# BreakTheBeta/Zonos_Vibes

Measured on AMD Instinct MI355X. Metric: real-time factor (44kHz audio s/compute s) + DAC tokens/s/GPU, Zonos-transformer, higher is better.
Workload: dtype bf16; 1 GPU; C2: batch=1 per GPU, Lc=160, 861 frames (10.00 s audio), greedy + rep. penalty, EOS suppressed, + DAC decode; global_batch=1, seq_len=1030, parallelism=dp1 (utterance-sharded), decode_steps=869

## Files before the change

### zonos_vibes_amd/csrc/zmi_gemv_impl.h

```cpp
#pragma once
#include <algorithm>
#include "zmi_common.h"
#include "zmi_kernels.h"
#include "zmi_gemv_row.h"
#include "zmi_rownorm.h"

namespace zmi_gemv {

constexpr int PRO_PLAIN = 0, PRO_LN = 1, PRO_ADDLN = 2, PRO_GRMS = 3;
constexpr int PRO_GRMSG = 4;
constexpr size_t LDS_MAX = 160 * 1024;

__device__ __forceinline__ void dma_piece(const bf16_t* gsrc, bf16_t* ldp) {
  const unsigned ldst =
      __builtin_amdgcn_readfirstlane((unsigned)(size_t)(__attribute__((address_space(3))) void*)ldp);
  unsigned keep;
  asm volatile("s_mov_b32 %0, m0\n\ts_mov_b32 m0, %2\n\ts_nop 0\n\tglobal_load_lds_dwordx4 %1, off\n\t"
               "s_mov_b32 m0, %0"
               : "=&s"(keep)
               : "v"(gsrc), "s"(ldst)
               : "memory");
}

template <int K>
struct Img {
  static constexpr int XROW = K + 8, GROW = K + 8;
  __host__ __device__ static constexpr bool grms(int pro) { return pro == PRO_GRMS || pro == PRO_GRMSG; }
  __host__ __device__ static constexpr size_t aux_off(int rows) { return (size_t)rows * XROW * 2; }
  __host__ __device__ static constexpr size_t gamma_off(int rows, int pro) {
    return aux_off(rows) + (size_t)rows * (pro == PRO_ADDLN ? XROW * 2 : (grms(pro) ? GROW * 4 : 0));
  }
  __host__ __device__ static constexpr size_t red_off(int rows, int pro) {
    return gamma_off(rows, pro) + (size_t)K * ((pro == PRO_LN || pro == PRO_ADDLN) ? 4 : (grms(pro) ? 2 : 0));
  }
  __host__ __device__ static constexpr size_t bytes(int rows, int nwv, int rt, int pro) {
    return red_off(rows, pro) + (size_t)nwv * 8 * rt * 4;
  }
  struct View {
    bf16_t *xs, *xa, *gam, *bet;
    float *xg, *red;
  };
  __device__ static View carve(char* smem, int rows, int pro) {
    char *aux = smem + aux_off(rows), *gamma = smem + gamma_off(rows, pro);
    return {reinterpret_cast<bf16_t*>(smem), reinterpret_cast<bf16_t*>(aux), reinterpret_cast<bf16_t*>(gamma),
            reinterpret_cast<bf16_t*>(gamma) + K, reinterpret_cast<float*>(aux),
            reinterpret_cast<float*>(smem + red_off(rows, pro))};
  }
};
template <int K>
using View = typename Img<K>::View;

#ifdef ZMI_GEMV_STAMPS
#define ZMI_GSTAMP(i)                                                                              \
  do {                                                                                             \
    __builtin_amdgcn_sched_barrier(0);                                                             \
    if (threadIdx.x == 0 && a.diag)                                                                \
      reinterpret_cast<unsigned long long*>(a.diag)[((size_t)a.reserved * 4096 + blockIdx.x) * 8 + (i)] = \
          __builtin_amdgcn_s_memrealtime();                                                        \
    __builtin_amdgcn_sched_barrier(0);                                                             \
  } while (0)
#else
#define ZMI_GSTAMP(i) \
  do {                \
  } while (0)
#endif

struct QkvFuse {
  uint64_t* gran;
  int gran_stride;
  int og_off = 0, of_off = 0, hkv = 0;
  const int* pos = nullptr;
  unsigned* err = nullptr;
  int l2_cols = 0;
};

__device__ __forceinline__ const float2* rope_pair(const ZmiGemvArgs& a, int q_pos, int n) {
  const int qcols = a.hq * a.hd, d = (n < qcols ? n : n - qcols) % a.hd;
  return reinterpret_cast<const float2*>(a.rope + ((size_t)q_pos * (a.hd >> 1) + (d >> 1)) * 2);
}

template <int EPI, int RT, int FUSE, class Sum>
__device__ __forceinline__ void epilogue(const ZmiGemvArgs& a, const Sum& colsum, int lane, int rows, int row0,
                                         int g, const uint32_t (&res_pre)[(8 * RT + 63) / 64], int q_pos, int q_kvr,
                                         const QkvFuse& fz, unsigned act_rows = ~0u, const float2* rope_pre = nullptr) {
  constexpr int NE = (8 * RT + 63) / 64;
  const int col0 = g * 8;
  if (EPI == ZMI_EPI_STORE && FUSE == 2) {
#pragma unroll
    for (int i = 0; i < NE; ++i) {
      const int e = lane + 64 * i, r = e >> 3, c = e & 7, n = col0 + c;
      const bool ok = r < rows && n < a.n_valid;
      const uint32_t hv = ok ? f2bf(colsum(c, r)) : 0u;
      const uint32_t nb = (uint32_t)__shfl_down((int)hv, 1);
      if (ok) {
        const size_t m = (size_t)(row0 + r);
        reinterpret_cast<bf16_t*>(a.out)[m * a.ldo + n] = (bf16_t)hv;
        const int pos = a.row_pos[m];
        if ((c & 1) == 0 && pos >= 0)
          st_xc64(fz.gran + m * fz.gran_stride + (n >> 1), (uint64_t)(hv | (nb << 16)) | ((uint64_t)(unsigned)(pos + 1) << 32),
                  n < fz.l2_cols);
      }
    }
  } else if (EPI == ZMI_EPI_STORE || EPI == ZMI_EPI_RESIDUAL || EPI == ZMI_EPI_F32 || EPI == ZMI_EPI_LOGITS) {
#pragma unroll
    for (int i = 0; i < NE; ++i) {
      const int e = lane + 64 * i, r = e >> 3, c = e & 7, n = col0 + c;
      if (r >= rows || n >= a.n_valid || !((act_rows >> r) & 1u)) continue;
      const float v = colsum(c, r);
      const size_t m = (size_t)(row0 + r);
      if (EPI == ZMI_EPI_F32) {
        reinterpret_cast<float*>(a.out)[m * a.ldo + n] = v;
      } else if (EPI == ZMI_EPI_STORE) {
        reinterpret_cast<bf16_t*>(a.out)[m * a.ldo + n] = (bf16_t)f2bf(v);
      } else if (EPI == ZMI_EPI_RESIDUAL) {
        reinterpret_cast<bf16_t*>(a.out)[m * a.ldo + n] = (bf16_t)f2bf(bf2f(res_pre[i]) + bfround(v));
      } else {
        const int cbk = n / 1026, vv = n - cbk * 1026;
        reinterpret_cast<float*>(a.out)[(m * 9 + cbk) * 1026 + vv] = bfround(v);
      }
    }
  } else if (EPI == ZMI_EPI_SWIGLU) {
    const int r = lane >> 2, c = lane & 3;
    if (r < rows) {
      const float y = bfround(colsum(c, r));
      const float gt = bfround(colsum(c + 4, r));
      const float sg = bfround(gt / (1.0f + expf(-gt)));
      reinterpret_cast<bf16_t*>(a.out)[(size_t)(row0 + r) * a.ldo + g * 4 + c] = (bf16_t)f2bf(y * sg);
    }
  } else if (EPI == ZMI_EPI_QKV) {
    const int r = lane >> 2, c = (lane & 3) * 2;
    if (r < rows && q_pos >= 0 && q_pos < a.smax) {
      const int n = col0 + c;
      const int qcols = a.hq * a.hd, kcols = a.hkv * a.hd;
      float x0 = bfround(colsum(c, r)), x1 = bfround(colsum(c + 1, r));
      if (n < qcols + kcols) {
        const float2 cs = rope_pre ? *rope_pre : *rope_pair(a, q_pos, n);
        const float co = cs.x, si = cs.y;
        const float r0 = x0 * co - x1 * si;
        const float r1 = x1 * co + x0 * si;
        x0 = r0;
        x1 = r1;
      }
      const uint32_t packed = f2bf(x0) | (f2bf(x1) << 16);
      int gkh = 0, gslot = 0;
      if (n < qcols) {
        *reinterpret_cast<uint32_t*>(reinterpret_cast<bf16_t*>(a.out) + (size_t)(row0 + r) * a.ldo + n) = packed;
        const int gq = a.hq / a.hkv;
        gkh = n / (gq * a.hd);
        gslot = (n - gkh * gq * a.hd) >> 1;
      } else if (n < qcols + kcols) {
        const int nn = n - qcols, kh = nn / a.hd, d = nn - kh * a.hd;
        const size_t o = (((size_t)q_kvr * a.hkv + kh) * a.smax + q_pos) * a.hd + d;
        *reinterpret_cast<uint32_t*>(reinterpret_cast<bf16_t*>(a.k_cache) + o) = packed;
        gkh = kh;
        gslot = (a.hq / a.hkv) * (a.hd >> 1) + (d >> 1);
      } else {
        const int nn = n - qcols - kcols, kh = nn / a.hd, d = nn - kh * a.hd;
        bf16_t* vt = reinterpret_cast<bf16_t*>(a.v_cache) + (((size_t)q_kvr * a.hkv + kh) * a.hd + d) * a.smax + q_pos;
        vt[0] = (bf16_t)(packed & 0xffffu);
        vt[a.smax] = (bf16_t)(packed >> 16);
        gkh = kh;
        gslot = (a.hq / a.hkv + 1) * (a.hd >> 1) + (d >> 1);
      }
      if (FUSE)
        st_wt64(fz.gran + ((size_t)(row0 + r) * a.hkv + gkh) * fz.gran_stride + gslot,
                (uint64_t)packed | ((uint64_t)(unsigned)(q_pos + 1) << 32));
    }
  }
}

template <int K, int PRO, int NWV>
__device__ __forceinline__ void stage_rows(const ZmiGemvArgs& a, const View<K>& L, int wave, int lane,
                                           bool first, int s_row0, int s_rows) {
  constexpr int XROW = Img<K>::XROW, GROW = Img<K>::GROW;
  constexpr bool GRMS = Img<K>::grms(PRO), AUX = PRO == PRO_ADDLN || GRMS;
  constexpr int GB = (PRO == PRO_LN || PRO == PRO_ADDLN) ? 2 : (GRMS ? 1 : 0);
  constexpr int PPR = K / 512;
  const int n_x = PRO == PRO_GRMSG ? 0 : s_rows * PPR;
  constexpr int APR = GRMS ? 2 * PPR : PPR;
  const int n_a = AUX ? s_rows * APR : 0;
  const int n_pc = n_x + n_a + (first ? GB * PPR : 0);
  const bf16_t* s_X = reinterpret_cast<const bf16_t*>(a.X) + (size_t)s_row0 * a.ldx;
  const bf16_t* XA = AUX ? reinterpret_cast<const bf16_t*>(a.aux) + (size_t)s_row0 * a.ld_aux * (GRMS ? 2 : 1)
                         : nullptr;
  for (int pc = wave; pc < n_pc; pc += NWV) {
    if (pc < n_x) {
      const int r = pc / PPR, p = pc - r * PPR;
      dma_piece(s_X + (size_t)r * a.ldx + p * 512 + lane * 8, L.xs + r * XROW + p * 512);
    } else if (pc < n_x + n_a) {
      const int r = (pc - n_x) / APR, p = (pc - n_x) - r * APR;
      if (GRMS)
        dma_piece(XA + ((size_t)r * a.ld_aux + p * 256) * 2 + lane * 8,
                  reinterpret_cast<bf16_t*>(L.xg + r * GROW + p * 256));
      else
        dma_piece(XA + (size_t)r * a.ld_aux + p * 512 + lane * 8, L.xa + r * XROW + p * 512);
    } else {
      const int q = pc - n_x - n_a, which = q / PPR, p = q - which * PPR;
      const bf16_t* src = reinterpret_cast<const bf16_t*>(which ? a.ln_b : a.ln_w);
      dma_piece(src + p * 512 + lane * 8, (which ? L.bet : L.gam) + p * 512);
    }
  }
}

template <int EPI, int RT>
__device__ __forceinline__ void stage_epilogue_operands(const ZmiGemvArgs& a, bool ew, int lane, int rows, int row0,
                                                        int col0, uint32_t (&res_pre)[(8 * RT + 63) / 64], int& q_pos,
                                                        int& q_kvr) {
  constexpr int NE = (8 * RT + 63) / 64;
#pragma unroll
  for (int i = 0; i < NE; ++i) res_pre[i] = 0;
  q_pos = -1, q_kvr = 0;
  if (EPI == ZMI_EPI_RESIDUAL && ew) {
#pragma unroll
    for (int i = 0; i < NE; ++i) {
      const int e = lane + 64 * i, r = e >> 3, n = col0 + (e & 7);
      if (r < rows && n < a.n_valid)
        res_pre[i] = reinterpret_cast<const bf16_t*>(a.out)[(size_t)(row0 + r) * a.ldo + n];
    }
  }
  if (EPI == ZMI_EPI_QKV && ew && (lane >> 2) < rows) {
    q_pos = a.row_pos[row0 + (lane >> 2)];
    q_kvr = a.row_kv[row0 + (lane >> 2)];
  }
}

template <int K, int NWV>
__device__ __forceinline__ unsigned gather_attention_rows(const ZmiGemvArgs& a, const QkvFuse& fz, bf16_t* xs, int* qpos,
                                                          int rows, int row0, int tid) {
  constexpr int XROW = Img<K>::XROW;
  const int lane = tid & 63, wave = __builtin_amdgcn_readfirstlane(tid >> 6);
  if (tid < rows) qpos[tid] = fz.pos[row0 + tid];
  __syncthreads();
  unsigned act_rows = 0u;
  for (int r = 0; r < rows; ++r) act_rows |= (qpos[r] >= 0 ? 1u : 0u) << r;
  const int n_units = rows * fz.hkv;
  if (wave == 0) {
    for (unsigned spins = 0;; ++spins) {
      bool ok = false;
      for (int u0 = 0; u0 < n_units; u0 += 8) {
        const int u = u0 + (lane >> 3), qp = u < n_units ? qpos[u / fz.hkv] : -1;
        const bool up = qp < 0 || (uint32_t)(ld_wt64(fz.gran + (size_t)(row0 * fz.hkv + u) * fz.gran_stride + fz.of_off +
                                                        (lane & 7)) >> 32) == (uint32_t)qp + 1u;
        float f = up ? 1.f : 0.f;
        f = fmaxf(f, dpp_mov<DPP_XOR1>(f));
        f = fmaxf(f, dpp_mov<DPP_XOR2>(f));
        f = fmaxf(f, dpp_mov<DPP_HALF_MIRROR>(f));
        ok = ok || (u < n_units && f > 0.f);
      }
      if (__any(ok)) break;
      if (spins > (1u << 18)) {
        if (lane == 0) __hip_atomic_store(fz.err, 1u, __ATOMIC_RELAXED, __HIP_MEMORY_SCOPE_AGENT);
        break;
      }
      __builtin_amdgcn_s_sleep(2);
    }
  }
  ZMI_GSTAMP(7);
  __syncthreads();
  constexpr int GPT = 4;
  for (int e0 = tid; e0 < n_units * 256; e0 += GPT * NWV * 64) {
    uint64_t gv[GPT];
    int gq[GPT];
    unsigned need = 0;
#pragma unroll
    for (int i = 0; i < GPT; ++i) {
      const int e = e0 + NWV * 64 * i;
      gq[i] = e < n_units * 256 ? qpos[(e >> 8) / fz.hkv] : -1;
      gv[i] = 0ull;
      if (gq[i] >= 0) need |= 1u << i;
    }
    for (unsigned spins = 0; need; ++spins) {
#pragma unroll
      for (int i = 0; i < GPT; ++i)
        if ((need >> i) & 1)
          gv[i] = ld_wt64(fz.gran + (size_t)(row0 * fz.hkv + ((e0 + NWV * 64 * i) >> 8)) * fz.gran_stride + fz.og_off +
                          ((e0 + NWV * 64 * i) & 255));
#pragma unroll
      for (int i = 0; i < GPT; ++i)
        if (((need >> i) & 1) && (uint32_t)(gv[i] >> 32) == (uint32_t)gq[i] + 1u) need &= ~(1u << i);
      if (!need) break;
      if (spins > (1u << 18)) {
        __hip_atomic_store(fz.err, 1u, __ATOMIC_RELAXED, __HIP_MEMORY_SCOPE_AGENT);
        break;
      }
      __builtin_amdgcn_s_sleep(1);
    }
#pragma unroll
    for (int i = 0; i < GPT; ++i) {
      const int e = e0 + NWV * 64 * i;
      if (e < n_units * 256) {
        const int u = e >> 8, j = e & 255, r = u / fz.hkv, kh = u - r * fz.hkv;
        *reinterpret_cast<uint32_t*>(xs + r * XROW + kh * 512 + 2 * j) = gq[i] >= 0 ? (uint32_t)gv[i] : 0u;
      }
    }
  }
  return act_rows;
}

template <int K, int RT, int NWV, bool ADD>
__device__ __forceinline__ void ln_statistics(const ZmiGemvArgs& a, const View<K>& L, int rows, int wave, int lane) {
  constexpr int XROW = Img<K>::XROW, NQ = ln_parts(K), CPQ = ln_chunks(K);
  float* part = L.red;
  const int ntask = rows * NQ;
  auto pass = [&](int task, float mean, bool sq) {
    const int r = task / NQ, q = task - r * NQ;
    float t = 0.f;
#pragma unroll
    for (int i = 0; i < CPQ; ++i) {
      const int off = r * XROW + ln_chunk_off(K, q, lane, i);
      const uint4 xv = ld_chunk(L.xs + off);
      if constexpr (ADD)
        t += addln_chunk_sum(xv, ld_chunk(L.xa + off), mean, sq);
      else
        t += ln_chunk_sum(xv, mean, sq);
    }
    return wave_sum(t);
  };
  for (int task = wave; task < ntask; task += NWV) {
    const float v = pass(task, 0.f, false);
    if (lane == 0) part[task] = v;
  }
  __syncthreads();
#if defined(ZMI_LN_STAMP) && ZMI_LN_STAMP == 1
  ZMI_GSTAMP(7);
#endif
  for (int task = wave; task < ntask; task += NWV) {
    const float mean = ln_combine<NQ>(part + (task / NQ) * NQ) / (float)K;
    const float v = pass(task, mean, true);
    if (lane == 0) part[RT * NQ + task] = v;
  }
  __syncthreads();
#if defined(ZMI_LN_STAMP) && ZMI_LN_STAMP == 2
  ZMI_GSTAMP(7);
#endif
}

template <int K, int RT, int NWV>
__device__ __forceinline__ void prologue_layernorm(const ZmiGemvArgs& a, const View<K>& L, int rows, int wave, int lane) {
  constexpr int XROW = Img<K>::XROW, NQ = ln_parts(K), CPQ = ln_chunks(K);
  ln_statistics<K, RT, NWV, false>(a, L, rows, wave, lane);
  for (int task = wave; task < rows * NQ; task += NWV) {
    const int r = task / NQ, q = task - r * NQ;
    const float mean = ln_combine<NQ>(L.red + r * NQ) / (float)K;
    const float rstd = 1.0f / sqrtf(ln_combine<NQ>(L.red + RT * NQ + r * NQ) / (float)K + a.eps), nbias = -mean * rstd;
#pragma unroll
    for (int i = 0; i < CPQ; ++i) {
      const int off = ln_chunk_off(K, q, lane, i);
      bf16_t* xp = L.xs + r * XROW + off;
      st_chunk(xp, ln_apply(ld_chunk(xp), ld_chunk(L.gam + off), ld_chunk(L.bet + off), rstd, nbias));
    }
  }
  __syncthreads();
}

template <int K, int RT, int NWV>
__device__ __forceinline__ void prologue_add_layernorm(const ZmiGemvArgs& a, const View<K>& L, int rows,
                                                       int row0, bool wres, int wave, int lane) {
  constexpr int XROW = Img<K>::XROW, NQ = ln_parts(K), CPQ = ln_chunks(K);
  ln_statistics<K, RT, NWV, true>(a, L, rows, wave, lane);
  for (int task = wave; task < rows * NQ; task += NWV) {
    const int r = task / NQ, q = task - r * NQ;
    const float mean = ln_combine<NQ>(L.red + r * NQ) / (float)K;
    const float rstd = 1.0f / sqrtf(ln_combine<NQ>(L.red + RT * NQ + r * NQ) / (float)K + a.eps);
#pragma unroll
    for (int i = 0; i < CPQ; ++i) {
      const int off = ln_chunk_off(K, q, lane, i);
      bf16_t* hp = L.xs + r * XROW + off;
      const AddLnChunk o = addln_apply(ld_chunk(hp), ld_chunk(L.xa + r * XROW + off), ld_chunk(L.gam + off),
                                       ld_chunk(L.bet + off), mean, rstd);
      st_chunk(hp, o.y);
      if (wres) st_chunk(reinterpret_cast<bf16_t*>(a.res_out) + (size_t)(row0 + r) * a.ld_aux + off, o.s);
    }
  }
  __syncthreads();
}

template <int K, int RT, int NWV, int PRO>
__device__ __forceinline__ void prologue_gated_rmsnorm(const ZmiGemvArgs& a, const View<K>& L, int rows,
                                                       int wave, int lane) {
  constexpr int XROW = Img<K>::XROW, GROW = Img<K>::GROW, NQ = ln_parts(K), CPQ = ln_chunks(K);
  float* part = L.red;
  const int ntask = rows * NQ;
  auto load_g = [&](int r, int off, float (&g)[8]) {
    uint32_t y[4] = {0u, 0u, 0u, 0u};
    if constexpr (PRO == PRO_GRMS) {
      const uint4 yv = *reinterpret_cast<const uint4*>(L.xs + r * XROW + off);
      y[0] = yv.x; y[1] = yv.y; y[2] = yv.z; y[3] = yv.w;
    }
    float gz[8];
    load_gate(L.xg + r * GROW + off, gz);
#pragma unroll
    for (int e = 0; e < 8; ++e) g[e] = PRO == PRO_GRMSG ? gz[e] : gate_elem(y, gz, e);
  };
  for (int task0 = wave; task0 < ntask; task0 += 2 * NWV) {
    float t[2];
#pragma unroll
    for (int u = 0; u < 2; ++u) {
      const int task = min(task0 + u * NWV, ntask - 1);
      const int r = task / NQ, q = task - r * NQ;
      t[u] = 0.f;
#pragma unroll
      for (int i = 0; i < CPQ; ++i) {
        float g[8];
        load_g(r, ln_chunk_off(K, q, lane, i), g);
        t[u] = grms_chunk_sq(g, t[u]);
      }
    }
#pragma unroll
    for (int u = 0; u < 2; ++u) t[u] = wave_sum(t[u]);
    if (lane == 0) {
      part[task0] = t[0];
      if (task0 + NWV < ntask) part[task0 + NWV] = t[1];
    }
  }
  __syncthreads();
  for (int task0 = wave; task0 < ntask; task0 += 2 * NWV) {
    uint4 res[2][CPQ];
#pragma unroll
    for (int u = 0; u < 2; ++u) {
      const int task = min(task0 + u * NWV, ntask - 1);
      const int r = task / NQ, q = task - r * NQ;
      const float rstd = 1.0f / sqrtf(ln_combine<NQ>(part + r * NQ) / (float)K + a.eps);
#pragma unroll
      for (int i = 0; i < CPQ; ++i) {
        const int off = ln_chunk_off(K, q, lane, i);
        const uint4 gw = *reinterpret_cast<const uint4*>(L.gam + off);
        float g[8];
        load_g(r, off, g);
        res[u][i] = grms_apply(g, gw, rstd);
      }
    }
#pragma unroll
    for (int u = 0; u < 2; ++u) {
      const int task = task0 + u * NWV;
      if (task < ntask) {
        const int r = task / NQ, q = task - r * NQ;
        bf16_t* yr = L.xs + r * XROW;
#pragma unroll
        for (int i = 0; i < CPQ; ++i) *reinterpret_cast<uint4*>(yr + ln_chunk_off(K, q, lane, i)) = res[u][i];
      }
    }
  }
  __syncthreads();
}

template <int G, int W, int NL, int RT, int PRO, int EPI, int NTW, int FUSE = 0, int FMT = ZMI_WFMT_BF16>
__device__ __forceinline__ void gemv_body(const ZmiGemvArgs& a, int n_cb, int n_rt, int b, char* smem,
                                          const QkvFuse& fz, int rpw = 1) {
  constexpr int K = W * NL * 64;
  constexpr int KC = K / 64;
  constexpr int NWV = G * W;
  constexpr int XROW = Img<K>::XROW;
  constexpr bool F8 = FMT == ZMI_WFMT_FP8;
  constexpr int CHB = F8 ? 512 : 1024;
  constexpr int NWL = F8 ? NL / 2 : NL;
  static_assert(FMT == ZMI_WFMT_BF16 || F8, "weight format");
  static_assert(!F8 || (NL % 2 == 0 && FUSE == 0 && (PRO == PRO_PLAIN || PRO == PRO_LN)),
                "fp8 weights: the MLP projections' plain / LayerNorm launches");
  static_assert(RT == 8 || RT == 16, "row tile");
  static_assert(!FUSE || EPI == ZMI_EPI_QKV || EPI == ZMI_EPI_STORE || FUSE == 3, "in-launch hand-off: QKV or plain store");
  static_assert(FUSE != 2 || NTW, "the store hand-off runs on single-tile (decode) launches");
  static_assert(FUSE != 3 || (NTW && (EPI == ZMI_EPI_RESIDUAL || EPI == ZMI_EPI_STORE) && PRO == PRO_PLAIN && K == 2048 &&
                              RT == 16),
                "the gathered-input form is zmi_attn_block's out_proj role (one tile, plain, residual or store epilogue)");

  const auto [cb, rg] = block_pos(b, n_rt, rpw);
  if (cb >= n_cb) return;
  ZMI_GSTAMP(0);
  int rt = rg * rpw;
  const int rt_end = min(n_rt, rt + rpw);
  int row0 = rt * RT;
  int rows = min(RT, a.M - row0);
  const View<K> L = Img<K>::carve(smem, a.M < RT ? a.M : RT, PRO);

  const int tid = threadIdx.x, lane = tid & 63;
  const int wave = __builtin_amdgcn_readfirstlane(tid >> 6);
  const int gi = wave / W, wk = wave - gi * W;
  const int ngroups = a.N >> 3;
  const int g_raw = cb * G + gi;
  const bool g_ok = g_raw < ngroups;
  const int g = g_ok ? g_raw : ngroups - 1;
  const int col0 = g * 8;
  const bool ew = (wk == 0) && g_ok;
  constexpr int NE = (8 * RT + 63) / 64;
  uint32_t res_pre[NE];
  int q_pos = -1, q_kvr = 0;
  unsigned act_rows = ~0u;

  if (FUSE != 3) stage_rows<K, PRO, NWV>(a, L, wave, lane, true, row0, rows);
  stage_epilogue_operands<EPI, RT>(a, ew, lane, rows, row0, col0, res_pre, q_pos, q_kvr);
  uint2 wexp = {0u, 0u};
  if constexpr (F8) {
    if (ew) wexp = *reinterpret_cast<const uint2*>(reinterpret_cast<const char*>(a.w_exp) + col0);
  }
  __builtin_amdgcn_sched_barrier(0);
  u32x4_t wf[NWL];
  load_weights_m8<NWL, NTW ? 2 : 0>(reinterpret_cast<const char*>(a.W) + ((size_t)g * KC + wk * NL) * CHB, NL * CHB,
                                    lane, wf);
  __builtin_amdgcn_sched_barrier(0);
  ZMI_GSTAMP(1);
  asm volatile("s_waitcnt vmcnt(%0)" ::"n"(NWL) : "memory");
  if constexpr (F8) {
    wexp.x = __builtin_amdgcn_readfirstlane(wexp.x);
    wexp.y = __builtin_amdgcn_readfirstlane(wexp.y);
  }
  float2 rope_cs = {1.f, 0.f};
  if (EPI == ZMI_EPI_QKV && NTW && ew && (lane >> 2) < rows && q_pos >= 0 && q_pos < a.smax) {
    const int n = col0 + (lane & 3) * 2;
    if (n < a.hq * a.hd + a.hkv * a.hd) rope_cs = *rope_pair(a, q_pos, n);
  }
  __builtin_amdgcn_sched_barrier(0);
  if constexpr (FUSE == 3)
    act_rows = gather_attention_rows<K, NWV>(a, fz, L.xs, reinterpret_cast<int*>(L.red), rows, row0, tid);
  for (;;) {
    __builtin_amdgcn_s_barrier();
    __builtin_amdgcn_sched_barrier(0);
    ZMI_GSTAMP(2);
    if constexpr (PRO == PRO_LN) prologue_layernorm<K, RT, NWV>(a, L, rows, wave, lane);
    if constexpr (PRO == PRO_ADDLN)
      prologue_add_layernorm<K, RT, NWV>(a, L, rows, row0, a.res_out != nullptr && cb == 0, wave, lane);
    if constexpr (PRO == PRO_GRMS || PRO == PRO_GRMSG) prologue_gated_rmsnorm<K, RT, NWV, PRO>(a, L, rows, wave, lane);
    ZMI_GSTAMP(3);

    f32x4_t acc0 = {0.f, 0.f, 0.f, 0.f}, acc1 = {0.f, 0.f, 0.f, 0.f};
    chain_m8<NL, F8>(L.xs + min(lane & 15, rows - 1) * XROW + wk * NL * 64 + (lane >> 4) * 8, wf, acc0, acc1);
    ZMI_GSTAMP(4);
    const SegPos sp = segment_pos<false>(lane);
#pragma unroll
    for (int q = 0; q < 4; ++q) {
      const float v = segment_value<false>(acc0, acc1, q);
      if (sp.live && sp.rb + q < RT) L.red[(wave * 8 + sp.c) * RT + sp.rb + q] = v;
    }
    __syncthreads();
    ZMI_GSTAMP(5);
    if (!NTW && rt + 1 < rt_end) {
      const int n_row0 = (rt + 1) * RT;
      stage_rows<K, PRO, NWV>(a, L, wave, lane, false, n_row0, min(RT, a.M - n_row0));
    }
    if (ew)
      epilogue<EPI, RT, FUSE>(a, ColSum<W, RT, F8>{L.red + gi * W * 8 * RT, wexp}, lane, rows, row0, g, res_pre, q_pos,
                              q_kvr, fz, act_rows, (EPI == ZMI_EPI_QKV && NTW) ? &rope_cs : nullptr);
    ZMI_GSTAMP(6);
    if (NTW || ++rt >= rt_end) break;
    __syncthreads();
    row0 = rt * RT;
    rows = min(RT, a.M - row0);
    stage_epilogue_operands<EPI, RT>(a, ew, lane, rows, row0, col0, res_pre, q_pos, q_kvr);
    asm volatile("s_waitcnt vmcnt(0)" ::: "memory");
  }
}

template <int G, int W, int NL, int RT, int PRO, int EPI, int NTW>
__global__ __launch_bounds__(G * W * 64) void gemv_kernel(const ZmiGemvArgs a, int n_cb, int n_rt, int rpw) {
  extern __shared__ __attribute__((aligned(16))) char smem[];
  gemv_body<G, W, NL, RT, PRO, EPI, NTW>(a, n_cb, n_rt, blockIdx.x, smem, QkvFuse{nullptr, 0}, rpw);
}
template <int G, int W, int NL, int RT, int PRO, int EPI, int NTW>
__global__ __launch_bounds__(G * W * 64) void gemv_kernel_f8(const ZmiGemvArgs a, int n_cb, int n_rt, int rpw) {
  extern __shared__ __attribute__((aligned(16))) char smem[];
  gemv_body<G, W, NL, RT, PRO, EPI, NTW, 0, ZMI_WFMT_FP8>(a, n_cb, n_rt, blockIdx.x, smem, QkvFuse{nullptr, 0}, rpw);
}

template <int FMT, int... A>
constexpr auto gemv_fn() {
  if constexpr (FMT == ZMI_WFMT_FP8)
    return &gemv_kernel_f8<A...>;
  else
    return &gemv_kernel<A...>;
}

#define ZMI_WAIT_VM(n) __builtin_amdgcn_s_waitcnt(((n) & 15) | (((n) >> 4) << 14) | 0x0F70)

constexpr int GR_G = 8, GR_RT = 16, GR_XROW = 2048 + 8;
constexpr size_t GR_RED = (size_t)2 * GR_RT * GR_XROW * 2;
constexpr size_t GR_OPS = GR_RED + (size_t)GR_G * 4 * 8 * GR_RT * 4;
constexpr size_t GR_CNT = GR_OPS + 2 * 2048;
constexpr size_t GR_LDS = GR_CNT + 16;

__device__ __forceinline__ void dma_dword(const void* gsrc, void* ldp) {
  const unsigned ldst =
      __builtin_amdgcn_readfirstlane((unsigned)(size_t)(__attribute__((address_space(3))) void*)ldp);
  unsigned keep;
  asm volatile("s_mov_b32 %0, m0\n\ts_mov_b32 m0, %2\n\ts_nop 0\n\tglobal_load_lds_dword %1, off\n\t"
               "s_mov_b32 m0, %0"
               : "=&s"(keep)
               : "v"(gsrc), "s"(ldst)
               : "memory");
}

template <int EPI, int GPW, bool DN = false>
__global__ __launch_bounds__(GR_G * 4 / GPW * 64 / (DN ? 2 : 1)) void gemm_rows_kernel(const ZmiGemvArgs a, int n_cb,
                                                                                       int n_rt, int rpw) {
  constexpr int W = 4, NL = 8, RT = GR_RT, K = 2048, KC = K / 64, XROW = GR_XROW, NE = 2;
  constexpr int NGS = DN ? GR_G / 2 / GPW : GR_G / GPW, NWV = NGS * W;
  static_assert(!DN || GPW == 1, "dense pairs: one pair per wave");
  constexpr int NDW = NWV / 2, PPW = RT * (K / 512) / NDW;
  static_assert(NDW >= GR_G, "the epilogue waves and the DMA waves are disjoint");
  constexpr int EP = EPI == ZMI_EPI_RESIDUAL ? 2 : (EPI == ZMI_EPI_QKV ? 1 : 0);
  extern __shared__ __attribute__((aligned(16))) char smem[];
  bf16_t* xs = reinterpret_cast<bf16_t*>(smem);
  float* red = reinterpret_cast<float*>(smem + GR_RED);
  char* ops = smem + GR_OPS;
  unsigned* cnt = reinterpret_cast<unsigned*>(smem + GR_CNT);
  const BlockPos bp = block_pos(blockIdx.x, n_rt, rpw);
  const int cb = bp.cb, rg = bp.rg;
  if (cb >= n_cb) return;
  ZMI_GSTAMP(0);
  const int tid = threadIdx.x, lane = tid & 63;
  const int wave = __builtin_amdgcn_readfirstlane(tid >> 6);
  const int gs = wave % NGS, wk = wave / NGS;
  const int ngroups = a.N >> 3;
  int gg[GPW];
#pragma unroll
  for (int h = 0; h < GPW; ++h) gg[h] = min(cb * GR_G + gs + NGS * h, ngroups - 1);
  const int n_ew = min(GR_G, ngroups - cb * GR_G);
  const bool ew = wave < n_ew;
  const int eg = cb * GR_G + wave;
  const int t0 = rg * rpw;
  const int rt_end = min(n_rt, t0 + rpw);
  const bf16_t* X = reinterpret_cast<const bf16_t*>(a.X);
  const bool opw = EP && wave == NWV - 1;
  const bool dw = wave >= NDW;
  if (tid == 0) *cnt = 0;
  volatile __attribute__((address_space(3))) unsigned* lcnt = (volatile __attribute__((address_space(3))) unsigned*)cnt;

  auto dma_tile = [&](int t) {
    if (!dw) return;
    bf16_t* dst = xs + (t & 1) * RT * XROW;
#pragma unroll
    for (int i = 0; i < PPW; ++i) {
      const int pc = wave - NDW + NDW * i, r = pc >> 2, p = pc & 3;
      const int sr = min(t * RT + r, a.M - 1);
      dma_piece(X + (size_t)sr * a.ldx + p * 512 + lane * 8, dst + r * XROW + p * 512);
    }
    if (opw) {
      char* od = ops + (t & 1) * 2048;
      if (EPI == ZMI_EPI_RESIDUAL) {
#pragma unroll
        for (int i = 0; i < 2; ++i) {
          const int e = lane + 64 * i, r = e >> 3, gi = min(cb * GR_G + (e & 7), ngroups - 1);
          dma_piece(reinterpret_cast<const bf16_t*>(a.out) + (size_t)min(t * RT + r, a.M - 1) * a.ldo + gi * 8,
                    reinterpret_cast<bf16_t*>(od + i * 1024));
        }
      } else if (EPI == ZMI_EPI_QKV) {
        const int r = min(t * RT + (lane & 15), a.M - 1);
        dma_dword((lane & 16) ? a.row_kv + r : a.row_pos + r, od);
      }
    }
  };

  dma_tile(t0);
  if (t0 + 1 < rt_end) dma_tile(t0 + 1);
  __builtin_amdgcn_sched_barrier(0);
  u32x4_t wf[DN ? 2 : GPW][NL];
  if constexpr (DN) {
    const int grp = min(cb * GR_G + 2 * gs + dn_member(lane), ngroups - 1) - cb * GR_G;
    load_weights_dn<NL, 0>(reinterpret_cast<const char*>(a.W) + (size_t)cb * GR_G * KC * 1024, GR_G * KC * 1024,
                           (grp * KC + wk * NL) * 1024, lane, wf);
  } else {
#pragma unroll
    for (int h = 0; h < GPW; ++h)
      load_weights_m8<NL, 0>(reinterpret_cast<const char*>(a.W) + ((size_t)gg[h] * KC + wk * NL) * 1024, NL * 1024, lane,
                             wf[h]);
  }
  __builtin_amdgcn_sched_barrier(0);
  ZMI_WAIT_VM(0);
  __syncthreads();

  for (int t = t0;; ++t) {
    const int ti = t - t0;
    if (ti == 1) ZMI_GSTAMP(2);
    const int row0 = t * RT, rows = min(RT, a.M - row0);
    const bool more = t + 1 < rt_end;
    f32x4_t acc0[GPW], acc1[GPW];
#pragma unroll
    for (int h = 0; h < GPW; ++h) acc0[h] = acc1[h] = f32x4_t{0.f, 0.f, 0.f, 0.f};
    {
      const bf16_t* xa = xs + (t & 1) * RT * XROW + (lane & 15) * XROW + wk * NL * 64 + (lane >> 4) * 8;
      if constexpr (DN) {
        chain_dn<NL>(xa, wf, acc0[0], acc1[0]);
      } else {
#pragma unroll
        for (int h = 0; h < GPW; ++h) chain_m8<NL, false>(xa, wf[h], acc0[h], acc1[h]);
      }
    }
    if (ti == 0) ZMI_GSTAMP(1);
    if (ti == 1) ZMI_GSTAMP(3);
    if (ti > 0) {
      const unsigned want = (unsigned)(n_ew * ti);
      for (int spin = 0; *lcnt < want && spin < (1 << 20); ++spin)
        __builtin_amdgcn_s_sleep(1);
    }
    {
      const SegPos sp = segment_pos<DN>(lane);
#pragma unroll
      for (int h = 0; h < (DN ? 1 : GPW); ++h)
#pragma unroll
        for (int q = 0; q < 4; ++q) {
          const float v = segment_value<DN>(acc0[h], acc1[h], q);
          const int grp = DN ? 2 * gs + (sp.c >> 3) : gs + NGS * h;
          if (sp.live) red[((grp * W + wk) * 8 + (sp.c & 7)) * RT + sp.rb + q] = v;
        }
    }
    uint32_t res_pre[NE] = {0u, 0u};
    int q_pos = -1, q_kvr = 0;
    if (ew) {
      const char* od = ops + (t & 1) * 2048;
      if (EPI == ZMI_EPI_RESIDUAL) {
#pragma unroll
        for (int i = 0; i < NE; ++i) {
          const int e = lane + 64 * i, r = e >> 3, c = e & 7;
          res_pre[i] = *reinterpret_cast<const uint16_t*>(od + (r * GR_G + wave) * 16 + c * 2);
        }
      }
      if (EPI == ZMI_EPI_QKV && (lane >> 2) < rows) {
        q_pos = reinterpret_cast<const int*>(od)[lane >> 2];
        q_kvr = reinterpret_cast<const int*>(od)[16 + (lane >> 2)];
      }
    }
    if (dw) ZMI_WAIT_VM(0);
    __builtin_amdgcn_fence(__ATOMIC_RELEASE, "workgroup", "local");
    __builtin_amdgcn_s_barrier();
    __builtin_amdgcn_fence(__ATOMIC_ACQUIRE, "workgroup", "local");
    if (ti == 1) ZMI_GSTAMP(4);
    if (t + 2 < rt_end) dma_tile(t + 2);
    if (ew) {
      epilogue<EPI, RT, 0>(a, ColSum<W, RT>{red + wave * W * 8 * RT}, lane, rows, row0, eg, res_pre, q_pos, q_kvr,
                           QkvFuse{nullptr, 0});
      if (more && lane == 0) __hip_atomic_fetch_add(cnt, 1u, __ATOMIC_RELAXED, __HIP_MEMORY_SCOPE_WORKGROUP);
    }
    if (ti == 1) ZMI_GSTAMP(5);
    if (!more) break;
  }
  ZMI_GSTAMP(7);
}


inline int rows_per_wg(int n_cb, int n_rt, int target) {
  if (n_rt <= 1) return 1;
  const int n_rg = std::max(1, std::min(n_rt, target / std::max(1, n_cb)));
  return (n_rt + n_rg - 1) / n_rg;
}

struct Shape {
  int W, NL, RT;
};
inline bool shape_for(int K, Shape* s) {
  switch (K) {
    case 512: *s = {2, 4, 16}; return true;
    case 1024: *s = {4, 4, 16}; return true;
    case 2048: *s = {4, 8, 16}; return true;
    case 4096: *s = {4, 16, 16}; return true;
    case 8192: *s = {8, 16, 8}; return true;
  }
  return false;
}

inline int groups_for(const ZmiGemvArgs& a, const Shape& s) {
  if (a.groups > 0) return a.groups;
  if (a.K == 8192 && a.M > 4 && a.N / 8 >= 256) return 2;
  if (a.K == 2048 && a.M > 16 && a.N / 8 >= 256 && a.ln_w == nullptr && a.pro == ZMI_PRO_AUTO) return 4;
  return (a.K == 2048 && a.N / 8 >= 384 && (a.ln_w != nullptr || a.pro != ZMI_PRO_AUTO || a.M > 4)) ? 2 : 1;
}

inline bool rows_form(int M, int N) { return M > 64 || (M > 32 && N >= 3072) || N >= 8192; }
inline bool rows_launch(const ZmiGemvArgs& a) {
  return a.w_fmt == ZMI_WFMT_BF16 && a.K == 2048 && a.M > GR_RT && a.ln_w == nullptr && a.pro == ZMI_PRO_AUTO &&
         a.groups == 0 && zmi_option(ZMI_OPT_GEMM_ROWS) && rows_form(a.M, a.N);
}

#define ZMI_GEMV_SHAPES(X) X(1, 2, 4, 16) X(1, 4, 4, 16) X(1, 4, 8, 16) X(2, 4, 8, 16) X(1, 4, 16, 16) X(1, 8, 16, 8) X(2, 8, 16, 8)

constexpr bool pro_built(int K, int epi, int pro, bool f8) {
  if (pro == PRO_ADDLN) return !f8 && (K == 512 || K == 2048) && epi != ZMI_EPI_RESIDUAL && epi != ZMI_EPI_F32;
  if (pro == PRO_GRMS || pro == PRO_GRMSG) return !f8 && (K == 1024 || K == 4096) && epi == ZMI_EPI_STORE;
  return !f8 || K != 4096;
}

inline size_t img_bytes(int K, int rows, int nwv, int rt, int pro) {
  switch (K) {
    case 512: return Img<512>::bytes(rows, nwv, rt, pro);
    case 1024: return Img<1024>::bytes(rows, nwv, rt, pro);
    case 2048: return Img<2048>::bytes(rows, nwv, rt, pro);
    case 4096: return Img<4096>::bytes(rows, nwv, rt, pro);
    default: return Img<8192>::bytes(rows, nwv, rt, pro);
  }
}

inline bool form_for(const ZmiGemvArgs& a, int epi, ZmiGemvForm* f) {
  Shape sh;
  if (!shape_for(a.K, &sh)) return false;
  const bool f8 = a.w_fmt == ZMI_WFMT_FP8;
  if (f8 && epi != ZMI_EPI_SWIGLU && epi != ZMI_EPI_RESIDUAL && epi != ZMI_EPI_F32) return false;
  if (rows_launch(a)) {
    const int n_cb = (a.N / 8 + GR_G - 1) / GR_G, n_rt = (a.M + GR_RT - 1) / GR_RT;
    *f = {(zmi_option(ZMI_OPT_GEMM_ROWS) & 2) ? ZMI_FORM_ROWS_DENSE : ZMI_FORM_ROWS, GR_G, 4, 8, GR_RT, 0, PRO_PLAIN,
          n_cb, n_rt, rows_per_wg(n_cb, n_rt, zmi_cu_count())};
    return true;
  }
  const int g = groups_for(a, sh);
  const int pro = a.pro != ZMI_PRO_AUTO ? a.pro : (a.ln_w != nullptr ? PRO_LN : PRO_PLAIN);
  const int ntw = a.M <= sh.RT;
  bool built = g == 4 && sh.W == 4 && sh.NL == 8 && sh.RT == 16 && !ntw && pro == PRO_PLAIN;
#define ZMI_SHAPE(G_, W_, NL_, RT_) built = built || (g == G_ && sh.W == W_ && sh.NL == NL_ && sh.RT == RT_);
  ZMI_GEMV_SHAPES(ZMI_SHAPE)
#undef ZMI_SHAPE
  if (!built) return false;
  if (!pro_built(a.K, epi, pro, f8) || (pro == PRO_GRMSG && !ntw)) return false;
  if (img_bytes(a.K, a.M < sh.RT ? a.M : sh.RT, g * sh.W, sh.RT, pro) > LDS_MAX) return false;
  const int n_cb = (a.N / 8 + g - 1) / g, n_rt = (a.M + sh.RT - 1) / sh.RT;
  *f = {ZMI_FORM_BODY, g, sh.W, sh.NL, sh.RT, ntw, pro, n_cb, n_rt, rows_per_wg(n_cb, n_rt, a.K == 8192 ? 256 : 512)};
  return true;
}

template <int G, int W, int NL, int RT, int PRO, int EPI, int NTW, int FMT = ZMI_WFMT_BF16>
hipError_t launch_p(const ZmiGemvArgs& a, hipStream_t s, const ZmiGemvForm& f) {
  constexpr int K = W * NL * 64;
  auto fn = gemv_fn<FMT, G, W, NL, RT, PRO, EPI, NTW>();
  size_t lds = Img<K>::bytes(a.M < RT ? a.M : RT, G * W, RT, PRO);
  const int64_t blocks = block_count(f.n_cb, f.n_rt, f.rpw);
  if (NTW && zmi_option(ZMI_OPT_GEMV_SPREAD)) {
    int64_t per_cu = (blocks + zmi_cu_count() - 1) / zmi_cu_count();
    if (zmi_option(ZMI_OPT_GEMV_SPREAD) > 1) per_cu = std::min<int64_t>(per_cu, zmi_option(ZMI_OPT_GEMV_SPREAD));
    if (per_cu < 8) lds = std::max(lds, LDS_MAX / (size_t)(per_cu + 1) + 1024);
  }
  if (lds > 64 * 1024) {
    static const hipError_t attr =
        hipFuncSetAttribute(reinterpret_cast<const void*>(fn), hipFuncAttributeMaxDynamicSharedMemorySize,
                            (int)LDS_MAX);
    if (attr != hipSuccess) return attr;
  }
  if (blocks > 0x7fffffff) return hipErrorInvalidValue;
  hipLaunchKernelGGL(fn, dim3((unsigned)blocks), dim3(G * W * 64), lds, s, a, f.n_cb, f.n_rt, f.rpw);
  return hipGetLastError();
}

template <int G, int W, int NL, int RT, int PRO, int EPI, int FMT = ZMI_WFMT_BF16>
hipError_t launch_tiles(const ZmiGemvArgs& a, hipStream_t s, const ZmiGemvForm& f) {
  return f.ntw ? launch_p<G, W, NL, RT, PRO, EPI, 1, FMT>(a, s, f) : launch_p<G, W, NL, RT, PRO, EPI, 0, FMT>(a, s, f);
}

template <int G, int W, int NL, int RT, int EPI, int FMT>
hipError_t launch_g(const ZmiGemvArgs& a, hipStream_t s, const ZmiGemvForm& f) {
  constexpr int K = W * NL * 64;
  constexpr bool F8 = FMT == ZMI_WFMT_FP8;
  if constexpr (pro_built(K, EPI, PRO_ADDLN, F8))
    if (f.pro == PRO_ADDLN) return launch_tiles<G, W, NL, RT, PRO_ADDLN, EPI>(a, s, f);
  if constexpr (pro_built(K, EPI, PRO_GRMS, F8)) {
    if (f.pro == PRO_GRMS) return launch_tiles<G, W, NL, RT, PRO_GRMS, EPI>(a, s, f);
    if (f.pro == PRO_GRMSG && f.ntw) return launch_p<G, W, NL, RT, PRO_GRMSG, EPI, 1>(a, s, f);
  }
  if constexpr (pro_built(K, EPI, PRO_LN, F8)) {
    if (f.pro == PRO_LN) return launch_tiles<G, W, NL, RT, PRO_LN, EPI, FMT>(a, s, f);
    if (f.pro == PRO_PLAIN) return launch_tiles<G, W, NL, RT, PRO_PLAIN, EPI, FMT>(a, s, f);
  }
  return hipErrorInvalidValue;
}

template <int EPI, int GPW, bool DN>
hipError_t launch_rows(const ZmiGemvArgs& a, hipStream_t s, const ZmiGemvForm& f) {
  auto fn = gemm_rows_kernel<EPI, GPW, DN>;
  const int64_t blocks = block_count(f.n_cb, f.n_rt, f.rpw);
  static const hipError_t attr = hipFuncSetAttribute(reinterpret_cast<const void*>(fn),
                                                     hipFuncAttributeMaxDynamicSharedMemorySize, (int)LDS_MAX);
  if (attr != hipSuccess) return attr;
  if (blocks > 0x7fffffff) return hipErrorInvalidValue;
  hipLaunchKernelGGL(fn, dim3((unsigned)blocks), dim3(GR_G * 4 / GPW * 64 / (DN ? 2 : 1)), GR_LDS, s, a, f.n_cb, f.n_rt,
                     f.rpw);
  return hipGetLastError();
}

template <int EPI, int FMT>
hipError_t launch_shape(const ZmiGemvArgs& a, hipStream_t s, const ZmiGemvForm& f) {
  if (f.G == 4) return launch_p<4, 4, 8, 16, PRO_PLAIN, EPI, 0, FMT>(a, s, f);
#define ZMI_SHAPE(G_, W_, NL_, RT_) \
  if (f.G == G_ && f.W == W_ && f.NL == NL_ && f.RT == RT_) return launch_g<G_, W_, NL_, RT_, EPI, FMT>(a, s, f);
  ZMI_GEMV_SHAPES(ZMI_SHAPE)
#undef ZMI_SHAPE
  return hipErrorInvalidValue;
}

template <int EPI>
hipError_t launch(const ZmiGemvArgs& a, hipStream_t s) {
  ZmiGemvForm f;
  if (!form_for(a, EPI, &f)) return hipErrorInvalidValue;
  if (f.kind == ZMI_FORM_ROWS_DENSE) return launch_rows<EPI, 1, true>(a, s, f);
  if (f.kind == ZMI_FORM_ROWS) return launch_rows<EPI, 2, false>(a, s, f);
  if (a.w_fmt == ZMI_WFMT_FP8) {
    if constexpr (EPI == ZMI_EPI_SWIGLU || EPI == ZMI_EPI_RESIDUAL || EPI == ZMI_EPI_F32)
      return launch_shape<EPI, ZMI_WFMT_FP8>(a, s, f);
    return hipErrorInvalidValue;
  }
  return launch_shape<EPI, ZMI_WFMT_BF16>(a, s, f);
}

}
```

Measured before the change: 12.77 x realtime (audio s / wall s, all GPUs).

## Split LayerNorm gamma/beta DMA wait to overlap with statistics pass

Issues the gamma/beta LDS DMA after the X/aux rows and waits only on X before computing LayerNorm statistics, deferring the gamma/beta vmcnt wait until after the variance pass. The barrier between passes becomes an LDS-only wait plus s_barrier. For QKV epilogues, row positions are loaded through uniform scalar loads so they don't sit in the vector-memory counter. It also adds an optional register-held LayerNorm path and a diagnostic stamp, both off by default. The gain is limited to a small prologue latency, and it depends on exact vmcnt ordering, which is fragile.

```diff
diff --git a/zonos_vibes_amd/csrc/zmi_gemv_impl.h b/zonos_vibes_amd/csrc/zmi_gemv_impl.h
--- a/zonos_vibes_amd/csrc/zmi_gemv_impl.h
+++ b/zonos_vibes_amd/csrc/zmi_gemv_impl.h
@@ -64,6 +64,21 @@
   do {                \
   } while (0)
 #endif
+#if defined(ZMI_GEMV_STAMPS) && defined(ZMI_LN_STAMP) && ZMI_LN_STAMP == 3
+#define ZMI_GWHERE()                                                                                          \
+  do {                                                                                                        \
+    if (threadIdx.x == 0 && a.diag)                                                                           \
+      reinterpret_cast<unsigned long long*>(a.diag)[((size_t)(a.reserved + 1) * 4096 + blockIdx.x) * 8] =     \
+          ((unsigned long long)__builtin_amdgcn_s_getreg(20 | (3 << 11)) << 32) |                             \
+          __builtin_amdgcn_s_getreg(4 | (31 << 11));                                                          \
+  } while (0)
+#else
+#define ZMI_GWHERE() \
+  do {               \
+  } while (0)
+#endif
+
+#define ZMI_WAIT_VM(n) __builtin_amdgcn_s_waitcnt(((n) & 15) | (((n) >> 4) << 14) | 0x0F70)
 
 struct QkvFuse {
   uint64_t* gran;
@@ -169,7 +184,7 @@
   }
 }
 
-template <int K, int PRO, int NWV>
+template <int K, int PRO, int NWV, bool GBOWN = false>
 __device__ __forceinline__ void stage_rows(const ZmiGemvArgs& a, const View<K>& L, int wave, int lane,
                                            bool first, int s_row0, int s_rows) {
   constexpr int XROW = Img<K>::XROW, GROW = Img<K>::GROW;
@@ -179,7 +194,7 @@
   const int n_x = PRO == PRO_GRMSG ? 0 : s_rows * PPR;
   constexpr int APR = GRMS ? 2 * PPR : PPR;
   const int n_a = AUX ? s_rows * APR : 0;
-  const int n_pc = n_x + n_a + (first ? GB * PPR : 0);
+  const int n_pc = n_x + n_a + ((first && !GBOWN) ? GB * PPR : 0);
   const bf16_t* s_X = reinterpret_cast<const bf16_t*>(a.X) + (size_t)s_row0 * a.ldx;
   const bf16_t* XA = AUX ? reinterpret_cast<const bf16_t*>(a.aux) + (size_t)s_row0 * a.ld_aux * (GRMS ? 2 : 1)
                          : nullptr;
@@ -200,6 +215,46 @@
       dma_piece(src + p * 512 + lane * 8, (which ? L.bet : L.gam) + p * 512);
     }
   }
+  if constexpr (GBOWN) {
+    if (first) {
+#pragma unroll
+      for (int q = wave; q < GB * PPR; q += NWV) {
+        const int which = q / PPR, p = q - which * PPR;
+        const bf16_t* src = reinterpret_cast<const bf16_t*>(which ? a.ln_b : a.ln_w);
+        dma_piece(src + p * 512 + lane * 8, (which ? L.bet : L.gam) + p * 512);
+      }
+    }
+  }
+}
+
+#ifndef ZMI_LN_SPLIT_WAIT
+#define ZMI_LN_SPLIT_WAIT 1
+#endif
+#ifndef ZMI_LN_SPLIT_FUSED
+#define ZMI_LN_SPLIT_FUSED 0
+#endif
+template <int K, int PRO, int NWV, int NTW>
+constexpr int ln_split_wait() {
+  constexpr int n_gb = 2 * (K / 512);
+  return (ZMI_LN_SPLIT_WAIT && NTW && (PRO == PRO_LN || PRO == PRO_ADDLN) && n_gb % NWV == 0) ? n_gb / NWV : 0;
+}
+template <int WAITN>
+__device__ __forceinline__ void pass_barrier() {
+  if constexpr (WAITN >= 0) {
+    asm volatile("s_waitcnt lgkmcnt(0)" ::: "memory");
+    __builtin_amdgcn_s_barrier();
+    asm volatile("" ::: "memory");
+  } else {
+    __syncthreads();
+  }
+}
+template <int WAITN>
+__device__ __forceinline__ void wait_gamma_beta() {
+  if constexpr (WAITN >= 0) {
+    __builtin_amdgcn_sched_barrier(0);
+    asm volatile("s_waitcnt vmcnt(%0)" ::"n"(WAITN) : "memory");
+    __builtin_amdgcn_sched_barrier(0);
+  }
 }
 
 template <int EPI, int RT>
@@ -223,6 +278,22 @@
     q_kvr = a.row_kv[row0 + (lane >> 2)];
   }
 }
+
+template <int RT>
+struct UniformPositions {
+  int pos[RT], kvr[RT];
+  __device__ __forceinline__ void load(const ZmiGemvArgs& a, int rows, int row0) {
+    typedef const __attribute__((address_space(4))) int* uniform_int_p;
+    const uniform_int_p rp = (uniform_int_p)(a.row_pos + row0), rk = (uniform_int_p)(a.row_kv + row0);
+#pragma unroll
+    for (int r = 0; r < RT; ++r) pos[r] = rp[min(r, rows - 1)], kvr[r] = rk[min(r, rows - 1)];
+  }
+  __device__ __forceinline__ void pick(int lane, int rows, int& q_pos, int& q_kvr) const {
+#pragma unroll
+    for (int r = 0; r < RT; ++r)
+      if (r < rows && (lane >> 2) == r) q_pos = pos[r], q_kvr = kvr[r];
+  }
+};
 
 template <int K, int NWV>
 __device__ __forceinline__ unsigned gather_attention_rows(const ZmiGemvArgs& a, const QkvFuse& fz, bf16_t* xs, int* qpos,
@@ -297,7 +368,7 @@
   return act_rows;
 }
 
-template <int K, int RT, int NWV, bool ADD>
+template <int K, int RT, int NWV, bool ADD, int WAITN = -1>
 __device__ __forceinline__ void ln_statistics(const ZmiGemvArgs& a, const View<K>& L, int rows, int wave, int lane) {
   constexpr int XROW = Img<K>::XROW, NQ = ln_parts(K), CPQ = ln_chunks(K);
   float* part = L.red;
@@ -320,7 +391,7 @@
     const float v = pass(task, 0.f, false);
     if (lane == 0) part[task] = v;
   }
-  __syncthreads();
+  pass_barrier<WAITN>();
 #if defined(ZMI_LN_STAMP) && ZMI_LN_STAMP == 1
   ZMI_GSTAMP(7);
 #endif
@@ -329,16 +400,76 @@
     const float v = pass(task, mean, true);
     if (lane == 0) part[RT * NQ + task] = v;
   }
+  wait_gamma_beta<WAITN>();
   __syncthreads();
 #if defined(ZMI_LN_STAMP) && ZMI_LN_STAMP == 2
   ZMI_GSTAMP(7);
 #endif
 }
 
-template <int K, int RT, int NWV>
+#ifndef ZMI_LN_HOLD
+#define ZMI_LN_HOLD 0
+#endif
+#ifndef ZMI_STAGE_FIRST
+#define ZMI_STAGE_FIRST 2
+#endif
+template <int K, int RT, int NWV, bool ADD, int WAITN>
+__device__ __forceinline__ void prologue_ln_held(const ZmiGemvArgs& a, const View<K>& L, int rows, int row0, bool wres,
+                                                 int wave, int lane) {
+  constexpr int XROW = Img<K>::XROW, NQ = ln_parts(K);
+  static_assert(ln_chunks(K) == 1, "one chunk per lane");
+  float* part = L.red;
+  const int task = wave, r = task / NQ, q = task - r * NQ;
+  const bool has = task < rows * NQ;
+  const int off = ln_chunk_off(K, q, lane, 0);
+  uint4 xv = {0u, 0u, 0u, 0u}, av = {0u, 0u, 0u, 0u};
+  if (has) {
+    xv = ld_chunk(L.xs + r * XROW + off);
+    if constexpr (ADD) av = ld_chunk(L.xa + r * XROW + off);
+  }
+  auto pass = [&](float mean, bool sq) {
+    float t = 0.f;
+    if constexpr (ADD)
+      t += addln_chunk_sum(xv, av, mean, sq);
+    else
+      t += ln_chunk_sum(xv, mean, sq);
+    return wave_sum(t);
+  };
+  if (has) {
+    const float v = pass(0.f, false);
+    if (lane == 0) part[task] = v;
+  }
+  pass_barrier<WAITN>();
+  float mean = 0.f;
+  if (has) {
+    mean = ln_combine<NQ>(part + r * NQ) / (float)K;
+    const float v = pass(mean, true);
+    if (lane == 0) part[RT * NQ + task] = v;
+  }
+  wait_gamma_beta<WAITN>();
+  __syncthreads();
+  if (has) {
+    const float rstd = 1.0f / sqrtf(ln_combine<NQ>(part + RT * NQ + r * NQ) / (float)K + a.eps);
+    bf16_t* xp = L.xs + r * XROW + off;
+    if constexpr (ADD) {
+      const AddLnChunk o = addln_apply(xv, av, ld_chunk(L.gam + off), ld_chunk(L.bet + off), mean, rstd);
+      st_chunk(xp, o.y);
+      if (wres) st_chunk(reinterpret_cast<bf16_t*>(a.res_out) + (size_t)(row0 + r) * a.ld_aux + off, o.s);
+    } else {
+      const float nbias = -mean * rstd;
+      st_chunk(xp, ln_apply(xv, ld_chunk(L.gam + off), ld_chunk(L.bet + off), rstd, nbias));
+    }
+  }
+  __syncthreads();
+}
+
+template <int K, int RT, int NWV, int WAITN = -1, bool HOLD = false>
 __device__ __forceinline__ void prologue_layernorm(const ZmiGemvArgs& a, const View<K>& L, int rows, int wave, int lane) {
   constexpr int XROW = Img<K>::XROW, NQ = ln_parts(K), CPQ = ln_chunks(K);
-  ln_statistics<K, RT, NWV, false>(a, L, rows, wave, lane);
+  if constexpr (HOLD && CPQ == 1) {
+    if (rows * NQ <= NWV) return prologue_ln_held<K, RT, NWV, false, WAITN>(a, L, rows, 0, false, wave, lane);
+  }
+  ln_statistics<K, RT, NWV, false, WAITN>(a, L, rows, wave, lane);
   for (int task = wave; task < rows * NQ; task += NWV) {
     const int r = task / NQ, q = task - r * NQ;
     const float mean = ln_combine<NQ>(L.red + r * NQ) / (float)K;
@@ -353,11 +484,14 @@
   __syncthreads();
 }
 
-template <int K, int RT, int NWV>
+template <int K, int RT, int NWV, int WAITN = -1, bool HOLD = false>
 __device__ __forceinline__ void prologue_add_layernorm(const ZmiGemvArgs& a, const View<K>& L, int rows,
                                                        int row0, bool wres, int wave, int lane) {
   constexpr int XROW = Img<K>::XROW, NQ = ln_parts(K), CPQ = ln_chunks(K);
-  ln_statistics<K, RT, NWV, true>(a, L, rows, wave, lane);
+  if constexpr (HOLD && CPQ == 1) {
+    if (rows * NQ <= NWV) return prologue_ln_held<K, RT, NWV, true, WAITN>(a, L, rows, row0, wres, wave, lane);
+  }
+  ln_statistics<K, RT, NWV, true, WAITN>(a, L, rows, wave, lane);
   for (int task = wave; task < rows * NQ; task += NWV) {
     const int r = task / NQ, q = task - r * NQ;
     const float mean = ln_combine<NQ>(L.red + r * NQ) / (float)K;
@@ -467,6 +601,7 @@
   const auto [cb, rg] = block_pos(b, n_rt, rpw);
   if (cb >= n_cb) return;
   ZMI_GSTAMP(0);
+  ZMI_GWHERE();
   int rt = rg * rpw;
   const int rt_end = min(n_rt, rt + rpw);
   int row0 = rt * RT;
@@ -487,11 +622,26 @@
   int q_pos = -1, q_kvr = 0;
   unsigned act_rows = ~0u;
 
-  if (FUSE != 3) stage_rows<K, PRO, NWV>(a, L, wave, lane, true, row0, rows);
-  stage_epilogue_operands<EPI, RT>(a, ew, lane, rows, row0, col0, res_pre, q_pos, q_kvr);
+  constexpr int GBW = (FUSE == 3 || (FUSE != 0 && !ZMI_LN_SPLIT_FUSED) || F8 || EPI == ZMI_EPI_RESIDUAL)
+                          ? 0
+                          : ln_split_wait<K, PRO, NWV, NTW>();
+  static_assert(NWL + GBW < 64, "vmcnt is a 6-bit count");
   uint2 wexp = {0u, 0u};
-  if constexpr (F8) {
-    if (ew) wexp = *reinterpret_cast<const uint2*>(reinterpret_cast<const char*>(a.w_exp) + col0);
+  if constexpr (GBW > 0) {
+    ZMI_WAIT_VM(0);
+#pragma unroll
+    for (int i = 0; i < NE; ++i) res_pre[i] = 0;
+    stage_rows<K, PRO, NWV, true>(a, L, wave, lane, true, row0, rows);
+    if constexpr (ZMI_STAGE_FIRST == 2 || (ZMI_STAGE_FIRST == 1 && FUSE == 1)) {
+      __builtin_amdgcn_sched_barrier(0);
+      __builtin_amdgcn_s_barrier();
+    }
+  } else {
+    if (FUSE != 3) stage_rows<K, PRO, NWV>(a, L, wave, lane, true, row0, rows);
+    stage_epilogue_operands<EPI, RT>(a, ew, lane, rows, row0, col0, res_pre, q_pos, q_kvr);
+    if constexpr (F8) {
+      if (ew) wexp = *reinterpret_cast<const uint2*>(reinterpret_cast<const char*>(a.w_exp) + col0);
+    }
   }
   __builtin_amdgcn_sched_barrier(0);
   u32x4_t wf[NWL];
@@ -499,7 +649,25 @@
                                     lane, wf);
   __builtin_amdgcn_sched_barrier(0);
   ZMI_GSTAMP(1);
-  asm volatile("s_waitcnt vmcnt(%0)" ::"n"(NWL) : "memory");
+  if constexpr (GBW > 0) {
+    UniformPositions<EPI == ZMI_EPI_QKV ? RT : 1> up;
+    if constexpr (EPI == ZMI_EPI_QKV) {
+      if (ew) up.load(a, rows, row0);
+      __builtin_amdgcn_sched_barrier(0);
+    }
+    ZMI_WAIT_VM(NWL + GBW);
+    __builtin_amdgcn_sched_barrier(0);
+#if defined(ZMI_LN_STAMP) && ZMI_LN_STAMP == 3
+    ZMI_GSTAMP(7);
+#endif
+    if constexpr (ZMI_LN_SPLIT_WAIT == 2) asm volatile("s_waitcnt vmcnt(%0)" ::"n"(NWL) : "memory");
+    if constexpr (EPI == ZMI_EPI_QKV) {
+      __builtin_amdgcn_sched_barrier(0);
+      if (ew) up.pick(lane, rows, q_pos, q_kvr);
+    }
+  } else {
+    asm volatile("s_waitcnt vmcnt(%0)" ::"n"(NWL) : "memory");
+  }
   if constexpr (F8) {
     wexp.x = __builtin_amdgcn_readfirstlane(wexp.x);
     wexp.y = __builtin_amdgcn_readfirstlane(wexp.y);
@@ -516,9 +684,11 @@
     __builtin_amdgcn_s_barrier();
     __builtin_amdgcn_sched_barrier(0);
     ZMI_GSTAMP(2);
-    if constexpr (PRO == PRO_LN) prologue_layernorm<K, RT, NWV>(a, L, rows, wave, lane);
+    constexpr int LNW = (GBW > 0 && ZMI_LN_SPLIT_WAIT == 1) ? NWL : -1;
+    constexpr bool HOLD = ZMI_LN_HOLD && FUSE == 1;
+    if constexpr (PRO == PRO_LN) prologue_layernorm<K, RT, NWV, LNW, HOLD>(a, L, rows, wave, lane);
     if constexpr (PRO == PRO_ADDLN)
-      prologue_add_layernorm<K, RT, NWV>(a, L, rows, row0, a.res_out != nullptr && cb == 0, wave, lane);
+      prologue_add_layernorm<K, RT, NWV, LNW, HOLD>(a, L, rows, row0, a.res_out != nullptr && cb == 0, wave, lane);
     if constexpr (PRO == PRO_GRMS || PRO == PRO_GRMSG) prologue_gated_rmsnorm<K, RT, NWV, PRO>(a, L, rows, wave, lane);
     ZMI_GSTAMP(3);
 
@@ -568,8 +738,6 @@
   else
     return &gemv_kernel<A...>;
 }
-
-#define ZMI_WAIT_VM(n) __builtin_amdgcn_s_waitcnt(((n) & 15) | (((n) >> 4) << 14) | 0x0F70)
 
 constexpr int GR_G = 8, GR_RT = 16, GR_XROW = 2048 + 8;
 constexpr size_t GR_RED = (size_t)2 * GR_RT * GR_XROW * 2;
```

Result: no change. 12.86 x realtime (audio s / wall s, all GPUs), median of 6 (+0.7%).
